# dmlc/difacto

Measured on AMD Instinct MI355X. Metric: examples/sec (FM SGD worker step, Criteo-shape, V_dim=64), higher is better.
Workload: dtype f32

## Files before the change

### difacto_amd/csrc/dfh_localize.hip

```cpp
#ifndef DFH_LOCALIZE_HIP_
#define DFH_LOCALIZE_HIP_
#include "dfh_internal.h"

namespace dfh {

constexpr int LOC_OVERSAMPLE = 8;
constexpr int LOC_MAX_BUCKETS = 1024;
constexpr int LOC_BIG_BUCKETS = 4096;
constexpr int LOC_AVG_BUCKET = 384;
constexpr int LOC_MIN_AVG = 48;
constexpr int LOC_MAX_AVG = 700;
constexpr int LOC_LDS_CAP = 1024;
#ifndef DFH_LOC_TILE
#define DFH_LOC_TILE 2048
#endif
#ifndef DFH_LOC_TILE_THREADS
#define DFH_LOC_TILE_THREADS 1024
#endif
constexpr int LOC_TILE = DFH_LOC_TILE;
constexpr int LOC_TILE_THREADS = DFH_LOC_TILE_THREADS;
constexpr int LOC_PER_THREAD = LOC_TILE / LOC_TILE_THREADS;
constexpr int LOC_SORT_THREADS = 256;
constexpr int LOC_EMIT_THREADS = 256;

struct LocView {
  const uint64_t* raw;
  uint32_t n;
  uint64_t max_index;
  int P;
  int bstride;
  int ntiles;
  int force_global;
  int tb;
  uint32_t nrows;
  const uint32_t* offset;
  const uint32_t* rowid;
  uint64_t* smp_key;
  uint32_t* smp_pos;
  uint32_t* smp_rank;
  uint64_t* spl_key;
  uint32_t* spl_pos;
  uint32_t* packed;
  uint32_t* run_off;
  uint32_t* btotal;
  uint32_t* bstart;
  uint64_t* bkeys;
  uint32_t* bpos;
  uint64_t* skeys;
  uint32_t* spos;
  uint64_t* first_key;
  uint64_t* last_key;
  uint32_t* nheads;
  uint32_t* lh;
  uint32_t* split_n;
};

struct SegListsOut {
  uint2* mid;
  SegEnt* mid_ent;
  uint2* hot;
  SegEnt* hot_ent;
  uint2* few;
  SegEnt* few_ent;
};

__device__ __forceinline__ uint64_t make_key(uint64_t id, uint64_t max_index) {
  const uint64_t m = (max_index == ~0ULL) ? (id == ~0ULL ? 0ULL : id) : id % max_index;
  return reverse_bytes(m);
}

constexpr int LOC_XCDS = 8;

__device__ __forceinline__ bool comp_less(uint64_t ka, uint32_t pa, uint64_t kb, uint32_t pb) {
  return ka < kb || (ka == kb && pa < pb);
}

template <bool MAX>
__device__ __forceinline__ uint32_t wave_inclusive(uint32_t x) {
#define DFH_DPP_STEP(ctrl, row_mask)                                                                      \
  {                                                                                                       \
    const uint32_t y = (uint32_t)__builtin_amdgcn_update_dpp(0, (int)x, ctrl, row_mask, 0xf, false);    \
    x = MAX ? max(x, y) : x + y;                                                                          \
  }
  DFH_DPP_STEP(0x111, 0xf)
  DFH_DPP_STEP(0x112, 0xf)
  DFH_DPP_STEP(0x114, 0xf)
  DFH_DPP_STEP(0x118, 0xf)
  DFH_DPP_STEP(0x142, 0xa)
  DFH_DPP_STEP(0x143, 0xc)
#undef DFH_DPP_STEP
  return x;
}

template <bool MAX, int NWAVES>
__device__ __forceinline__ uint32_t block_exclusive(uint32_t val, uint32_t* wtot , uint32_t* total) {
  static_assert(NWAVES <= 64, "one lane per wave");
  const int lane = (int)(threadIdx.x & 63);
  const int w = __builtin_amdgcn_readfirstlane((int)(threadIdx.x >> 6));
  const uint32_t s = wave_inclusive<MAX>(val);
  __syncthreads();
  if (lane == 63) wtot[w] = s;
  __syncthreads();
  const uint32_t x = wave_inclusive<MAX>(lane < NWAVES ? wtot[lane] : 0u);
  const uint32_t before = w ? (uint32_t)__builtin_amdgcn_readlane((int)x, w - 1) : 0u;
  if (total) *total = (uint32_t)__builtin_amdgcn_readlane((int)x, NWAVES - 1);
  const uint32_t prev = (uint32_t)__builtin_amdgcn_update_dpp(0, (int)s, 0x138, 0xf, 0xf, false);
  return MAX ? max(before, prev) : before + prev;
}
template <int NWAVES>
__device__ __forceinline__ uint32_t block_exclusive_scan(uint32_t val, uint32_t* wsum , uint32_t* total) {
  return block_exclusive<false, NWAVES>(val, wsum, total);
}
template <int NWAVES>
__device__ __forceinline__ uint32_t block_exclusive_max(uint32_t val, uint32_t* wmax , uint32_t* total) {
  return block_exclusive<true, NWAVES>(val, wmax, total);
}

__device__ __forceinline__ uint32_t ss_sample_pos(uint32_t t, uint32_t stride, uint32_t n) {
  const uint32_t j = (uint32_t)(splitmix64(t) >> 33) % stride;
  return min(t * stride + j, n - 1);
}

__global__ void __launch_bounds__(256) k_ss_sample(LocView v) {
  const uint32_t S = (uint32_t)v.P * LOC_OVERSAMPLE;
  const uint32_t stride = max(1u, v.n / S);
  for (uint32_t t = blockIdx.x * blockDim.x + threadIdx.x; t < S; t += gridDim.x * blockDim.x) {
    const uint32_t i = ss_sample_pos(t, stride, v.n);
    v.smp_key[t] = make_key(v.raw[i], v.max_index);
    v.smp_pos[t] = i << v.tb;
    v.smp_rank[t] = 0;
  }
}

__global__ void __launch_bounds__(256) k_ss_rank(LocView v) {
  __shared__ uint64_t ck[256];
  __shared__ uint32_t cp[256];
  const uint32_t S = (uint32_t)v.P * LOC_OVERSAMPLE;
  const uint32_t ntile = (S + 255) / 256;
  const uint32_t ti = blockIdx.x / ntile, tj = blockIdx.x % ntile;
  const uint32_t col = tj * 256 + threadIdx.x;
  ck[threadIdx.x] = col < S ? v.smp_key[col] : ~0ULL;
  cp[threadIdx.x] = col < S ? v.smp_pos[col] : ~0u;
  const uint32_t row = ti * 256 + threadIdx.x;
  const uint64_t mk = row < S ? v.smp_key[row] : 0;
  const uint32_t mp = row < S ? v.smp_pos[row] : 0;
  __syncthreads();
  const uint32_t lim = min(256u, S - tj * 256);
  uint32_t rank = 0;
#pragma unroll 8
  for (uint32_t j = 0; j < lim; ++j) {
    const bool less = comp_less(ck[j], cp[j], mk, mp) || (ck[j] == mk && cp[j] == mp && tj * 256 + j < row);
    rank += less ? 1u : 0u;
  }
  if (row < S && rank) atomicAdd(&v.smp_rank[row], rank);
}

__global__ void __launch_bounds__(256) k_loc_splitters(LocView v) {
  const uint32_t S = (uint32_t)v.P * LOC_OVERSAMPLE;
  for (uint32_t t = blockIdx.x * blockDim.x + threadIdx.x; t < S; t += gridDim.x * blockDim.x) {
    const uint32_t r = v.smp_rank[t];
    if (r > 0 && r % LOC_OVERSAMPLE == 0) {
      v.spl_key[r / LOC_OVERSAMPLE - 1] = v.smp_key[t];
      v.spl_pos[r / LOC_OVERSAMPLE - 1] = v.smp_pos[t];
    }
  }
}

constexpr int LOC_GATHER_ROWS = 1024;
constexpr int LOC_GATHER_SEGS = 4;
struct GatherSrc {
  int nseg;
  uint32_t seg_row0[LOC_GATHER_SEGS + 1];
  const uint32_t* src_off[LOC_GATHER_SEGS];
  const uint64_t* src_idx[LOC_GATHER_SEGS];
  const float* src_val[LOC_GATHER_SEGS];
  const uint32_t* h_rows;
  const uint32_t* h_off;
  const float* h_lab;
  const uint32_t* h_tile_row;
  uint64_t* dst_raw;
  float* dst_val;
  uint32_t* dst_off;
  float* dst_lab;
};
constexpr size_t loc_gather_smem() { return (size_t)(LOC_GATHER_ROWS + 1) * 4 + 4 + (size_t)LOC_GATHER_ROWS * 8; }
template <typename T>
__device__ __forceinline__ T loc_sel(const T (&a)[LOC_GATHER_SEGS], uint32_t sg) {
  T r = a[0];
#pragma unroll
  for (int x = 1; x < LOC_GATHER_SEGS; ++x) r = sg == (uint32_t)x ? a[x] : r;
  return r;
}

template <int MAXB>
constexpr size_t loc_count_smem() { return (size_t)MAXB * 16; }
template <int MAXB, int THREADS>
constexpr size_t loc_scatter_smem() { return (size_t)MAXB * 4 + (THREADS / 64) * 4; }
constexpr size_t loc_sort_smem() { return (size_t)LOC_LDS_CAP * 24 + 2 * (LOC_SORT_THREADS / 64) * 4; }
constexpr size_t loc_emit_smem() { return (2 * (LOC_EMIT_THREADS / 64) + 4) * 4; }

template <int MAXB, int THREADS, bool GATHER = false>
__device__ __forceinline__ void loc_count_block(const LocView& v, const uint32_t bid, const uint32_t nblk, char* smem,
                                                const GatherSrc* gp = nullptr) {
  constexpr int PER = LOC_TILE / THREADS;
  static_assert(PER * THREADS == LOC_TILE, "a tile is a whole number of elements per thread");
  uint64_t* sk = reinterpret_cast<uint64_t*>(smem);
  uint32_t* sp = reinterpret_cast<uint32_t*>(smem + (size_t)MAXB * 8);
  uint32_t* hist = sp + MAXB;
  const int P = v.P;
  for (int b = threadIdx.x; b < P; b += THREADS) {
    hist[b] = 0;
    sk[b] = b < P - 1 ? v.spl_key[b] : ~0ULL;
    sp[b] = b < P - 1 ? v.spl_pos[b] : ~0u;
  }
  const uint32_t base = bid * LOC_TILE;
  if (bid == 0 && threadIdx.x == 0 && v.split_n) *v.split_n = 0u;
  uint64_t key[PER];
  if (GATHER) {
    const GatherSrc& g = *gp;
    uint32_t* roff = reinterpret_cast<uint32_t*>(smem + loc_count_smem<MAXB>());
    uint64_t* rsrc = reinterpret_cast<uint64_t*>(roff + LOC_GATHER_ROWS + 2);
    const uint32_t row0 = g.h_tile_row[bid], row1 = g.h_tile_row[bid + 1];
    const uint32_t nr = min(row1, v.nrows - 1u) - row0 + 1u;
    for (uint32_t q = threadIdx.x; q <= nr; q += THREADS) roff[q] = g.h_off[row0 + q];
    for (uint32_t q = threadIdx.x; q < nr; q += THREADS) {
      const uint32_t r = row0 + q;
      uint32_t sg = 0;
#pragma unroll
      for (int x = 1; x < LOC_GATHER_SEGS; ++x) sg += (x < g.nseg && r >= g.seg_row0[x]) ? 1u : 0u;
      rsrc[q] = ((uint64_t)loc_sel(g.src_off, sg)[g.h_rows[r]] << 2) | sg;
    }
    __syncthreads();
#pragma unroll
    for (int e = 0; e < PER; ++e) {
      const uint32_t i = base + e * THREADS + threadIdx.x;
      key[e] = ~0ULL;
      if (i < v.n) {
        uint32_t lo = 0, hi = nr - 1u;
        while (lo < hi) {
          const uint32_t mid = (lo + hi + 1u) >> 1;
          if (roff[mid] <= i) lo = mid; else hi = mid - 1u;
        }
        const uint64_t sw = rsrc[lo];
        const uint32_t sg = (uint32_t)(sw & 3u);
        const size_t at = (size_t)(sw >> 2) + (i - roff[lo]);
        const uint64_t id = loc_sel(g.src_idx, sg)[at];
        g.dst_raw[i] = id;
        if (g.dst_val) {
          const float* sv = loc_sel(g.src_val, sg);
          g.dst_val[i] = sv ? sv[at] : 1.0f;
        }
        key[e] = make_key(id, v.max_index);
      }
    }
  } else {
#pragma unroll
    for (int e = 0; e < PER; ++e) {
      const uint32_t i = base + e * THREADS + threadIdx.x;
      key[e] = i < v.n ? make_key(v.raw[i], v.max_index) : ~0ULL;
    }
  }
  {
    uint32_t* __restrict__ rowid = const_cast<uint32_t*>(v.rowid);
    const uint32_t* __restrict__ offset = GATHER ? gp->h_off : v.offset;
    const uint32_t rpb = (v.nrows + nblk - 1) / nblk;
    const uint32_t r0 = bid * rpb, r1 = min(v.nrows, r0 + rpb);
    for (uint32_t r = r0 + threadIdx.x; r < r1; r += THREADS) {
      const uint32_t b0 = offset[r], e = offset[r + 1];
      if (GATHER) {
        gp->dst_off[r] = b0;
        gp->dst_lab[r] = gp->h_lab[r];
        if (r + 1 == v.nrows) gp->dst_off[r + 1] = e;
      }
      for (uint32_t j = b0; j < e; ++j) rowid[j] = r;
    }
  }
  __syncthreads();
  int lo[PER], hi[PER];
#pragma unroll
  for (int e = 0; e < PER; ++e) { lo[e] = 0; hi[e] = P - 1; }
  for (int step = P; step > 1; step = (step + 1) >> 1) {
#pragma unroll
    for (int e = 0; e < PER; ++e) {
      if (lo[e] < hi[e]) {
        const uint32_t i = base + e * THREADS + threadIdx.x;
        const int mid = (lo[e] + hi[e]) >> 1;
        if (comp_less(key[e], i << v.tb, sk[mid], sp[mid])) hi[e] = mid; else lo[e] = mid + 1;
      }
    }
  }
#pragma unroll
  for (int e = 0; e < PER; ++e) {
    const uint32_t i = base + e * THREADS + threadIdx.x;
    if (i < v.n) {
      const uint32_t r = atomicAdd(&hist[lo[e]], 1u);
      v.packed[i] = ((uint32_t)lo[e] << 16) | r;
    }
  }
  __syncthreads();
  for (int b = threadIdx.x; b < P; b += THREADS) {
    const uint32_t h = hist[b];
    v.run_off[bid * P + b] = h ? atomicAdd(&v.btotal[(bid & (LOC_XCDS - 1)) * MAXB + b], h) : 0u;
  }
}

template <int MAXB>
__global__ void __launch_bounds__(LOC_TILE_THREADS) k_loc_count(LocView v) {
  __shared__ __attribute__((aligned(16))) char smem[loc_count_smem<MAXB>()];
  loc_count_block<MAXB, LOC_TILE_THREADS>(v, blockIdx.x, gridDim.x, smem);
}
template <int MAXB>
__global__ void __launch_bounds__(LOC_TILE_THREADS) k_loc_count_gather(LocView v, GatherSrc g) {
  __shared__ __attribute__((aligned(16))) char smem[loc_count_smem<MAXB>() + loc_gather_smem()];
  loc_count_block<MAXB, LOC_TILE_THREADS, true>(v, blockIdx.x, gridDim.x, smem, &g);
}

constexpr int LOC_DESC_ROWS = 256;
__global__ void __launch_bounds__(LOC_DESC_ROWS) k_loc_describe(const uint32_t* __restrict__ src_off, const float* __restrict__ src_lab,
                                                                const uint32_t* __restrict__ h_rows, const uint32_t* __restrict__ h_base,
                                                                uint32_t n, uint32_t* __restrict__ dst_off, float* __restrict__ dst_lab,
                                                                int write_end) {
  __shared__ uint32_t wsum[LOC_DESC_ROWS / 64];
  const uint32_t q = blockIdx.x * LOC_DESC_ROWS + threadIdx.x;
  const bool in = q < n;
  const uint32_t r = h_rows[in ? q : n - 1u];
  const uint32_t lo = src_off[r], hi = src_off[r + 1u];
  const float lab = src_lab[r];
  const uint32_t len = in ? hi - lo : 0u;
  const uint32_t at = h_base[blockIdx.x] + block_exclusive_scan<LOC_DESC_ROWS / 64>(len, wsum, nullptr);
  if (in) {
    dst_off[q] = at;
    dst_lab[q] = lab;
    if (write_end && q + 1u == n) dst_off[n] = at + len;
  }
}


template <int MAXB, int THREADS>
__device__ __forceinline__ void loc_scatter_block(const LocView& v, const uint32_t bid, char* smem) {
  constexpr int PER = LOC_TILE / THREADS;
  constexpr int LOC_BPT = MAXB / THREADS;
  static_assert(LOC_BPT * THREADS == MAXB, "the scan of the bucket totals gives every thread the same number of buckets");
  uint32_t* off = reinterpret_cast<uint32_t*>(smem);
  uint32_t* wsum = off + MAXB;
  const int P = v.P;
  const uint32_t xcd = bid & (LOC_XCDS - 1);
  const uint32_t base = bid * LOC_TILE;
  const int b0 = threadIdx.x * LOC_BPT;
  uint32_t tt[LOC_BPT], ro[LOC_BPT];
  uint32_t sum = 0;
#pragma unroll
  for (int q = 0; q < LOC_BPT; ++q) {
    const int bb = min(b0 + q, P - 1);
    const uint32_t in = b0 + q < P ? 1u : 0u;
    tt[q] = 0;
    ro[q] = v.run_off[bid * P + bb];
#pragma unroll
    for (int x = 0; x < LOC_XCDS; ++x) {
      const uint32_t h = v.btotal[x * MAXB + bb];
      tt[q] += h;
      ro[q] += (x < (int)xcd ? 1u : 0u) * h;
    }
    tt[q] *= in;
    ro[q] *= in;
    sum += tt[q];
  }
  uint32_t total;
  uint32_t ex = block_exclusive_scan<THREADS / 64>(sum, wsum, &total);
#pragma unroll
  for (int q = 0; q < LOC_BPT; ++q) {
    if (b0 + q < P) {
      off[b0 + q] = ex + ro[q];
      if (bid == 0) v.bstart[b0 + q] = ex;
    }
    ex += tt[q];
  }
  if (bid == 0 && threadIdx.x == 0) v.bstart[P] = total;
  uint64_t raw[PER];
  uint32_t pk[PER], rw[PER];
#pragma unroll
  for (int e = 0; e < PER; ++e) {
    const uint32_t i = min(base + e * THREADS + threadIdx.x, v.n - 1);
    raw[e] = v.raw[i];
    pk[e] = v.packed[i];
    rw[e] = v.rowid[i];
  }
  __syncthreads();
#pragma unroll
  for (int e = 0; e < PER; ++e) {
    const uint32_t i = base + e * THREADS + threadIdx.x;
    if (i < v.n) {
      const uint32_t dst = off[pk[e] >> 16] + (pk[e] & 0xFFFFu);
      v.bkeys[dst] = make_key(raw[e], v.max_index);
      v.bpos[dst] = (i << v.tb) | (rw[e] & ((1u << v.tb) - 1u));
    }
  }
}

template <int MAXB>
__global__ void __launch_bounds__(LOC_TILE_THREADS) k_loc_scatter(LocView v) {
  __shared__ __attribute__((aligned(16))) char smem[loc_scatter_smem<MAXB, LOC_TILE_THREADS>()];
  loc_scatter_block<MAXB, LOC_TILE_THREADS>(v, blockIdx.x, smem);
}

template <int J>
__device__ __forceinline__ uint32_t loc_net_partner(uint32_t x) {
  static_assert(J == 1 || J == 2 || J == 4 || J == 8, "DPP reaches the partners inside a row of 16 lanes");
  if constexpr (J == 1) return (uint32_t)__builtin_amdgcn_mov_dpp((int)x, 0xB1, 0xf, 0xf, false);
  if constexpr (J == 2) return (uint32_t)__builtin_amdgcn_mov_dpp((int)x, 0x4E, 0xf, 0xf, false);
  if constexpr (J == 4) {
    const int y = __builtin_amdgcn_mov_dpp((int)x, 0x141, 0xf, 0xf, false);
    return (uint32_t)__builtin_amdgcn_mov_dpp(y, 0x1B, 0xf, 0xf, false);
  }
  return (uint32_t)__builtin_amdgcn_mov_dpp((int)x, 0x128, 0xf, 0xf, false);
}
constexpr uint64_t loc_net_keeps_max(int K, int J) {
  uint64_t m = 0;
  for (int i = 0; i < 64; ++i) m |= (uint64_t)(((i & J) != 0) != ((i & K) != 0)) << i;
  return m;
}
template <int K, int J>
__device__ __forceinline__ void loc_net_stage(uint32_t& klo, uint32_t& khi, uint32_t& tag) {
  uint32_t mlo, mhi;
  asm volatile("s_mov_b32 %0, %2\n\ts_mov_b32 %1, %3"
               : "=s"(mlo), "=s"(mhi)
               : "i"((int32_t)(uint32_t)loc_net_keeps_max(K, J)), "i"((int32_t)(uint32_t)(loc_net_keeps_max(K, J) >> 32)));
  const uint64_t mask = ((uint64_t)mhi << 32) | mlo;
  const bool keeps_max = __builtin_amdgcn_inverse_ballot_w64(mask);
  if constexpr (J >= 16) {
    uint32_t alo, ahi, at, blo, bhi, bt;
#define DFH_NET_SWAP(a, b, x)                                                                                       \
    {                                                                                                                 \
      const auto r = J == 16 ? __builtin_amdgcn_permlane16_swap(x, x, false, false) : __builtin_amdgcn_permlane32_swap(x, x, false, false); \
      a = r[0];                                                                                                       \
      b = r[1];                                                                                                       \
    }
    DFH_NET_SWAP(alo, blo, klo)
    DFH_NET_SWAP(ahi, bhi, khi)
    DFH_NET_SWAP(at, bt, tag)
#undef DFH_NET_SWAP
    const bool out_of_order = comp_less(((uint64_t)bhi << 32) | blo, bt, ((uint64_t)ahi << 32) | alo, at);
    const bool take_b = out_of_order != keeps_max;
    klo = take_b ? blo : alo;
    khi = take_b ? bhi : ahi;
    tag = take_b ? bt : at;
  } else {
    const uint32_t olo = loc_net_partner<J>(klo), ohi = loc_net_partner<J>(khi), ot = loc_net_partner<J>(tag);
    const bool partner_less = comp_less(((uint64_t)ohi << 32) | olo, ot, ((uint64_t)khi << 32) | klo, tag);
    const bool take = partner_less != keeps_max;
    klo = take ? olo : klo;
    khi = take ? ohi : khi;
    tag = take ? ot : tag;
  }
}
template <int K, int J>
__device__ __forceinline__ void loc_net_merge(uint32_t& klo, uint32_t& khi, uint32_t& tag) {
  loc_net_stage<K, J>(klo, khi, tag);
  if constexpr (J > 1) loc_net_merge<K, J / 2>(klo, khi, tag);
}
template <int K = 2>
__device__ __forceinline__ void loc_net_sort64(uint32_t& klo, uint32_t& khi, uint32_t& tag) {
  loc_net_merge<K, K / 2>(klo, khi, tag);
  if constexpr (K < 64) loc_net_sort64<K * 2>(klo, khi, tag);
}

__device__ __forceinline__ bool loc_sort_bucket_lds(const LocView& v, uint32_t beg, uint32_t n, uint64_t* ak, uint32_t* ap,
                                                    uint64_t* bk, uint32_t* bp) {
  const uint64_t* gk = v.bkeys + beg;
  const uint32_t* gp = v.bpos + beg;
  uint64_t* sk = bk;
  uint32_t* sp = bp;
  const uint32_t lane = threadIdx.x & 63;
  for (uint32_t c0 = (threadIdx.x >> 6) * 64; c0 < n; c0 += LOC_SORT_THREADS) {
    const uint32_t idx = c0 + lane;
    const bool valid = idx < n;
    const uint64_t mk = valid ? gk[idx] : ~0ULL;
    uint32_t klo = (uint32_t)mk, khi = (uint32_t)(mk >> 32);
    uint32_t mp = valid ? gp[idx] : ~0u;
    loc_net_sort64(klo, khi, mp);
    if (valid) {
      bk[idx] = ((uint64_t)khi << 32) | klo;
      bp[idx] = mp;
    }
  }
  __syncthreads();
  constexpr int E = LOC_LDS_CAP / LOC_SORT_THREADS;
  constexpr int G = 2;
  static_assert(E * LOC_SORT_THREADS == LOC_LDS_CAP && E % G == 0 && LOC_SORT_THREADS % 64 == 0,
                "a thread carries E elements of a full bucket, G at a time");
  uint64_t* dk = ak;
  uint32_t* dp = ap;
  uint32_t sh = 6;
  for (uint32_t L = 64; L < n; L <<= 1, ++sh) {
    for (int g = 0; g < E && g * LOC_SORT_THREADS < (int)n; g += G) {
      uint64_t mk[G];
      uint32_t mp[G], at[G], end[G];
#pragma unroll
      for (int e = 0; e < G; ++e) {
        const uint32_t idx = threadIdx.x + (g + e) * LOC_SORT_THREADS;
        const bool valid = idx < n;
        const uint32_t sib = ((idx >> sh) ^ 1u) << sh;
        mk[e] = valid ? sk[idx] : 0ULL;
        mp[e] = valid ? sp[idx] : 0u;
        at[e] = min(sib, n);
        end[e] = valid ? min(sib + L, n) : at[e];
      }
      for (uint32_t step = L; step; step >>= 1) {
        uint64_t ok[G];
        uint32_t op[G];
#pragma unroll
        for (int e = 0; e < G; ++e) {
          const uint32_t q = at[e] + step <= end[e] ? at[e] + step - 1u : 0u;
          ok[e] = sk[q];
          op[e] = sp[q];
        }
#pragma unroll
        for (int e = 0; e < G; ++e)
          if (at[e] + step <= end[e] && comp_less(ok[e], op[e], mk[e], mp[e])) at[e] += step;
      }
#pragma unroll
      for (int e = 0; e < G; ++e) {
        const uint32_t idx = threadIdx.x + (g + e) * LOC_SORT_THREADS;
        if (idx < n) {
          const uint32_t dst = idx + at[e] - min((idx & ~(L - 1u)) | L, n);
          dk[dst] = mk[e];
          dp[dst] = mp[e];
        }
      }
    }
    __syncthreads();
    uint64_t* tk = sk; sk = dk; dk = tk;
    uint32_t* tp = sp; sp = dp; dp = tp;
  }
  return sk == ak;
}
__device__ __forceinline__ void loc_sort_bucket_global(const LocView& v, uint32_t beg, uint32_t n) {
  uint64_t* xk = v.bkeys + beg;
  uint32_t* xp = v.bpos + beg;
  uint64_t* yk = v.skeys + beg;
  uint32_t* yp = v.spos + beg;
  const uint32_t lane = threadIdx.x & 63;
  for (uint32_t c0 = (threadIdx.x >> 6) * 64; c0 < n; c0 += LOC_SORT_THREADS) {
    const uint32_t idx = c0 + lane;
    const bool valid = idx < n;
    const uint64_t mk = valid ? xk[idx] : ~0ULL;
    const uint32_t mp = valid ? xp[idx] : ~0u;
    const uint32_t lim = min(64u, n - c0);
    uint32_t rank = 0;
    for (uint32_t j = 0; j < lim; ++j) rank += comp_less(xk[c0 + j], xp[c0 + j], mk, mp) ? 1u : 0u;
    if (valid) {
      yk[c0 + rank] = mk;
      yp[c0 + rank] = mp;
    }
  }
  __syncthreads();
  uint64_t* srck = yk; uint32_t* srcp = yp;
  uint64_t* dstk = xk; uint32_t* dstp = xp;
  for (uint32_t L = 64; L < n; L <<= 1) {
    for (uint32_t idx = threadIdx.x; idx < n; idx += blockDim.x) {
      const uint64_t mk = srck[idx];
      const uint32_t mp = srcp[idx];
      const uint32_t r = idx / L;
      const uint32_t pair_base = (r & ~1u) * L;
      const uint32_t sib = (r ^ 1u) * L;
      uint32_t lo = min(sib, n), hi = min(sib + L, n);
      const uint32_t sib_beg = lo;
      while (lo < hi) {
        const uint32_t mid = (lo + hi) >> 1;
        if (comp_less(srck[mid], srcp[mid], mk, mp)) lo = mid + 1; else hi = mid;
      }
      const uint32_t dst = pair_base + (idx - r * L) + (lo - sib_beg);
      dstk[dst] = mk;
      dstp[dst] = mp;
    }
    __syncthreads();
    uint64_t* tk = srck; srck = dstk; dstk = tk;
    uint32_t* tp = srcp; srcp = dstp; dstp = tp;
  }
  if (srck != yk) {
    for (uint32_t t = threadIdx.x; t < n; t += blockDim.x) {
      yk[t] = srck[t];
      yp[t] = srcp[t];
    }
  }
  __syncthreads();
}

struct BucketSummary {
  uint32_t nheads, lh;
  uint64_t first_key, last_key;
};
template <bool WRITE>
__device__ __forceinline__ BucketSummary loc_bucket_summary(const uint64_t* sk, const uint32_t* sp, uint32_t n, uint64_t* ok,
                                                            uint32_t* op, uint32_t (*red)[LOC_SORT_THREADS / 64]) {
  uint32_t cnt = 0, last = 0;
  uint32_t t0 = threadIdx.x;
  asm volatile("" : "+v"(t0));
  for (uint32_t t = t0; t < n; t += LOC_SORT_THREADS) {
    const uint64_t k = sk[t];
    if (WRITE) {
      ok[t] = k;
      op[t] = sp[t];
    }
    if (t + 1 < n && sk[t + 1] != k) {
      ++cnt;
      last = t + 1;
    }
  }
  cnt = (uint32_t)__builtin_amdgcn_readlane((int)wave_inclusive<false>(cnt), 63);
  last = (uint32_t)__builtin_amdgcn_readlane((int)wave_inclusive<true>(last), 63);
  if ((threadIdx.x & 63) == 0) {
    red[0][threadIdx.x >> 6] = cnt;
    red[1][threadIdx.x >> 6] = last;
  }
  __syncthreads();
  BucketSummary r;
  r.nheads = 1;
  r.lh = 0;
  r.first_key = 0;
  r.last_key = 0;
  if (threadIdx.x == 0) {
    for (int w = 0; w < LOC_SORT_THREADS / 64; ++w) {
      r.nheads += red[0][w];
      r.lh = max(r.lh, red[1][w]);
    }
    r.first_key = sk[0];
    r.last_key = sk[n - 1];
  }
  return r;
}

__device__ __forceinline__ void loc_sort_block(const LocView& v, const uint32_t bid, const uint32_t nblk, char* smem) {
  uint64_t* ak = reinterpret_cast<uint64_t*>(smem);
  uint64_t* bk = ak + LOC_LDS_CAP;
  uint32_t* ap = reinterpret_cast<uint32_t*>(bk + LOC_LDS_CAP);
  uint32_t* bp = ap + LOC_LDS_CAP;
  uint32_t (*red)[LOC_SORT_THREADS / 64] = reinterpret_cast<uint32_t (*)[LOC_SORT_THREADS / 64]>(bp + LOC_LDS_CAP);
  for (uint32_t b = bid; b < (uint32_t)v.P; b += nblk) {
    __syncthreads();
    const uint32_t beg = v.bstart[b], end = v.bstart[b + 1];
    const uint32_t n = end - beg;
    if (threadIdx.x < LOC_XCDS) v.btotal[threadIdx.x * v.bstride + b] = 0;
    if (n == 0) {
      if (threadIdx.x == 0) {
        v.nheads[b] = 0;
        v.lh[b] = 0;
        v.first_key[b] = 0;
        v.last_key[b] = 0;
      }
      continue;
    }
    BucketSummary sm;
    if (n <= LOC_LDS_CAP && !v.force_global) {
      const bool in_a = loc_sort_bucket_lds(v, beg, n, ak, ap, bk, bp);
      sm = loc_bucket_summary<true>(in_a ? ak : bk, in_a ? ap : bp, n, v.skeys + beg, v.spos + beg, red);
    } else {
      loc_sort_bucket_global(v, beg, n);
      sm = loc_bucket_summary<false>(v.skeys + beg, v.spos + beg, n, nullptr, nullptr, red);
    }
    if (threadIdx.x == 0) {
      v.nheads[b] = sm.nheads;
      v.lh[b] = sm.lh;
      v.first_key[b] = sm.first_key;
      v.last_key[b] = sm.last_key;
    }
  }
}
__global__ void __launch_bounds__(LOC_SORT_THREADS) k_loc_sort(LocView v) {
  extern __shared__ __attribute__((aligned(16))) char smem[];
  loc_sort_block(v, blockIdx.x, gridDim.x, smem);
}

template <int NW, bool PROBE>
__device__ __forceinline__ void loc_emit_bucket(const LocView& v, uint32_t b, uint32_t beg, uint32_t n, const uint64_t* sk,
                                                const uint32_t* sp, uint32_t cont, uint32_t ubase, uint32_t carry1,
                                                const float* __restrict__ value,
                                                uint64_t* __restrict__ feaids, uint32_t* __restrict__ col_ptr,
                                                uint32_t* __restrict__ index, uint32_t* __restrict__ s_row,
                                                float* __restrict__ s_val, uint32_t* __restrict__ d_U, const SegListsOut& sl,
                                                uint32_t* wsum, uint32_t* wmax, uint32_t* n_mid, uint32_t* n_hot,
                                                uint32_t* n_few, const TableView& tab, uint32_t* __restrict__ urow) {
  const uint32_t P = (uint32_t)v.P;
  const uint32_t moff = beg / (BWD_SMALL + 1) + 2 * b, hoff = beg / (BWD_MID + 1) + 2 * b, foff = beg / 2 + 2 * b;
  uint32_t run_heads = 0, run_max1 = carry1;
  for (uint32_t base = 0; base < n; base += blockDim.x) {
    const uint32_t t = base + threadIdx.x;
    const uint32_t i = beg + t;
    const bool valid = t < n;
    uint64_t key = 0;
    uint32_t tag = 0;
    bool head = false;
    if (valid) {
      key = sk[t];
      tag = sp[t];
      head = t == 0 ? !cont : key != sk[t - 1];
    }
    const uint32_t pos = tag >> v.tb;
    uint32_t nh, mx;
    const uint32_t ex = block_exclusive_scan<NW>(head ? 1u : 0u, wsum, &nh);
    const uint32_t pm = block_exclusive_max<NW>(head ? i + 1 : 0u, wmax, &mx);
    if (valid) {
      const uint32_t incl = run_heads + ex + (head ? 1u : 0u);
      const uint32_t uid = ubase + incl - 1;
      const uint32_t prev1 = max(run_max1, pm);
      if (head) {
        feaids[uid] = key;
        col_ptr[uid] = i;
        if (PROBE) urow[uid] = find_or_insert(tab, key);
        if (prev1) {
          const uint32_t len = i - (prev1 - 1);
          const SegEnt e = make_uint4(uid - 1, prev1 - 1, i, 0u);
          if (len > BWD_MID) sl.hot_ent[hoff + atomicAdd(n_hot, 1u)] = e;
          else if (len > BWD_SMALL) sl.mid_ent[moff + atomicAdd(n_mid, 1u)] = e;
          else if (len > 1) sl.few_ent[foff + atomicAdd(n_few, 1u)] = e;
        }
      }
      index[pos] = uid;
      uint32_t row = tag & ((1u << v.tb) - 1u);
      {
        const uint32_t step = 1u << v.tb;
        uint32_t lo = 0, hi = v.nrows > row ? (v.nrows - 1u - row) >> v.tb : 0u;
        while (lo < hi) {
          const uint32_t mid = (lo + hi + 1u) >> 1;
          if (v.offset[row + mid * step] <= pos) lo = mid; else hi = mid - 1u;
        }
        row += lo * step;
      }
      s_row[i] = row;
      if (value) s_val[i] = value[pos];
      if (i == v.n - 1) {
        *d_U = uid + 1;
        col_ptr[uid + 1] = v.n;
        const uint32_t lbeg = head ? i : prev1 - 1, len = v.n - lbeg;
        const SegEnt e = make_uint4(uid, lbeg, v.n, 0u);
        if (len > BWD_MID) sl.hot_ent[hoff + atomicAdd(n_hot, 1u)] = e;
        else if (len > BWD_SMALL) sl.mid_ent[moff + atomicAdd(n_mid, 1u)] = e;
        else if (len > 1) sl.few_ent[foff + atomicAdd(n_few, 1u)] = e;
      }
    }
    run_heads += nh;
    run_max1 = max(run_max1, mx);
  }
  if (P > 1) {
    const uint64_t N = v.n;
    const uint64_t m0 = max((uint64_t)beg * P / N + ((uint64_t)beg * P % N ? 1u : 0u), (uint64_t)1);
    const uint64_t e1 = (uint64_t)(beg + n) * P;
    const uint64_t m1 = min(e1 / N + (e1 % N ? 1u : 0u), (uint64_t)P);
    for (uint64_t m = m0 + threadIdx.x; m < m1; m += blockDim.x) {
      const uint32_t i = (uint32_t)(m * N / P);
      if ((i * (uint64_t)P + N - 1) / N == m) {
        v.spl_key[m - 1] = sk[i - beg];
        v.spl_pos[m - 1] = sp[i - beg];
      }
    }
  }
  __syncthreads();
  if (threadIdx.x == 0) {
    sl.mid[b] = make_uint2(*n_mid, moff);
    sl.hot[b] = make_uint2(*n_hot, hoff);
    sl.few[b] = make_uint2(*n_few, foff);
  }
}

struct EmitOut {
  const float* value;
  uint64_t* feaids;
  uint32_t* col_ptr;
  uint32_t* index;
  uint32_t* s_row;
  float* s_val;
  uint32_t* d_U;
  SegListsOut sl;
};

template <bool PROBE>
__device__ __forceinline__ void loc_emit_block(const LocView& v, const EmitOut& o, const TableView& tab, uint32_t* __restrict__ urow,
                                               const uint32_t bid, const uint32_t nblk, char* smem) {
  constexpr int NW = LOC_EMIT_THREADS / 64;
  uint32_t* wsum = reinterpret_cast<uint32_t*>(smem);
  uint32_t* wmax = wsum + NW;
  uint32_t& sh_cont = wmax[NW];
  uint32_t& n_mid = wmax[NW + 1];
  uint32_t& n_hot = wmax[NW + 2];
  uint32_t& n_few = wmax[NW + 3];
  const SegListsOut& sl = o.sl;
  const uint32_t P = (uint32_t)v.P;
  for (uint32_t b = bid; b < P; b += nblk) {
    __syncthreads();
    const uint32_t beg = v.bstart[b], end = v.bstart[b + 1];
    const uint32_t n = end - beg;
    if (threadIdx.x == 0) {
      n_mid = 0;
      n_hot = 0;
      n_few = 0;
      if (n == 0) {
        sl.mid[b] = make_uint2(0u, 0u);
        sl.hot[b] = make_uint2(0u, 0u);
        sl.few[b] = make_uint2(0u, 0u);
      }
    }
    if (n == 0) continue;
    uint32_t part = 0, carry1 = 0;
    for (uint32_t q0 = threadIdx.x; q0 <= b; q0 += LOC_EMIT_THREADS) {
      const uint32_t bq = v.bstart[q0], nq = v.bstart[q0 + 1] - bq;
      if (nq == 0) continue;
      int p = (int)q0 - 1;
      while (p >= 0 && v.bstart[p + 1] == v.bstart[p]) --p;
      const uint32_t c = (p >= 0 && v.first_key[q0] == v.last_key[p]) ? 1u : 0u;
      if (q0 == b) {
        sh_cont = c;
      } else {
        part += v.nheads[q0] - c;
        const uint32_t l = v.lh[q0];
        if (l > 0) carry1 = max(carry1, bq + l + 1);
        else if (!c) carry1 = max(carry1, bq + 1);
      }
    }
    uint32_t ubase, carry_all;
    block_exclusive_scan<NW>(part, wsum, &ubase);
    block_exclusive_max<NW>(carry1, wmax, &carry_all);
    __syncthreads();
    loc_emit_bucket<NW, PROBE>(v, b, beg, n, v.skeys + beg, v.spos + beg, sh_cont, ubase, carry_all, o.value, o.feaids, o.col_ptr,
                               o.index, o.s_row, o.s_val, o.d_U, sl, wsum, wmax, &n_mid, &n_hot, &n_few, tab, urow);
  }
}

template <bool PROBE>
__global__ void __launch_bounds__(LOC_EMIT_THREADS) k_loc_emit(LocView v, EmitOut o, TableView tab, uint32_t* __restrict__ urow) {
  __shared__ __attribute__((aligned(16))) char smem[loc_emit_smem()];
  loc_emit_block<PROBE>(v, o, tab, urow, blockIdx.x, gridDim.x, smem);
}

}
#endif
```

Baseline: 87.34 million.

## Sort 128-element runs per wave and merge all runs by rank in one pass

The in-LDS bucket sort now runs a two-register-per-lane bitonic network over 128-element runs instead of 64, with the cross-register stage done in-lane. The log-depth pairwise merge passes, each ending in a block barrier, are replaced by a single pass. In that pass each element finds its final position by binary-searching every other sorted run, then scatters directly to the output buffer. This removes the repeated merge rounds and barriers, but the per-element search cost now grows with the number of runs and padded sentinel entries are written to LDS.

```diff
diff --git a/difacto_amd/csrc/dfh_localize.hip b/difacto_amd/csrc/dfh_localize.hip
--- a/difacto_amd/csrc/dfh_localize.hip
+++ b/difacto_amd/csrc/dfh_localize.hip
@@ -419,14 +419,8 @@
   for (int i = 0; i < 64; ++i) m |= (uint64_t)(((i & J) != 0) != ((i & K) != 0)) << i;
   return m;
 }
-template <int K, int J>
-__device__ __forceinline__ void loc_net_stage(uint32_t& klo, uint32_t& khi, uint32_t& tag) {
-  uint32_t mlo, mhi;
-  asm volatile("s_mov_b32 %0, %2\n\ts_mov_b32 %1, %3"
-               : "=s"(mlo), "=s"(mhi)
-               : "i"((int32_t)(uint32_t)loc_net_keeps_max(K, J)), "i"((int32_t)(uint32_t)(loc_net_keeps_max(K, J) >> 32)));
-  const uint64_t mask = ((uint64_t)mhi << 32) | mlo;
-  const bool keeps_max = __builtin_amdgcn_inverse_ballot_w64(mask);
+template <int J, bool INV>
+__device__ __forceinline__ void loc_net_exchange(const bool keeps_max, uint32_t& klo, uint32_t& khi, uint32_t& tag) {
   if constexpr (J >= 16) {
     uint32_t alo, ahi, at, blo, bhi, bt;
 #define DFH_NET_SWAP(a, b, x)                                                                                       \
@@ -440,99 +434,119 @@
     DFH_NET_SWAP(at, bt, tag)
 #undef DFH_NET_SWAP
     const bool out_of_order = comp_less(((uint64_t)bhi << 32) | blo, bt, ((uint64_t)ahi << 32) | alo, at);
-    const bool take_b = out_of_order != keeps_max;
+    const bool take_b = INV ? out_of_order == keeps_max : out_of_order != keeps_max;
     klo = take_b ? blo : alo;
     khi = take_b ? bhi : ahi;
     tag = take_b ? bt : at;
   } else {
     const uint32_t olo = loc_net_partner<J>(klo), ohi = loc_net_partner<J>(khi), ot = loc_net_partner<J>(tag);
     const bool partner_less = comp_less(((uint64_t)ohi << 32) | olo, ot, ((uint64_t)khi << 32) | klo, tag);
-    const bool take = partner_less != keeps_max;
+    const bool take = INV ? partner_less == keeps_max : partner_less != keeps_max;
     klo = take ? olo : klo;
     khi = take ? ohi : khi;
     tag = take ? ot : tag;
   }
 }
 template <int K, int J>
-__device__ __forceinline__ void loc_net_merge(uint32_t& klo, uint32_t& khi, uint32_t& tag) {
-  loc_net_stage<K, J>(klo, khi, tag);
-  if constexpr (J > 1) loc_net_merge<K, J / 2>(klo, khi, tag);
+__device__ __forceinline__ void loc_net_stage(uint32_t& k0lo, uint32_t& k0hi, uint32_t& t0, uint32_t& k1lo, uint32_t& k1hi,
+                                              uint32_t& t1) {
+  if constexpr (J == 64) {
+    const bool swap = comp_less(((uint64_t)k1hi << 32) | k1lo, t1, ((uint64_t)k0hi << 32) | k0lo, t0);
+    const uint32_t lo = k0lo, hi = k0hi, t = t0;
+    k0lo = swap ? k1lo : lo;
+    k0hi = swap ? k1hi : hi;
+    t0 = swap ? t1 : t;
+    k1lo = swap ? lo : k1lo;
+    k1hi = swap ? hi : k1hi;
+    t1 = swap ? t : t1;
+  } else {
+    uint32_t mlo, mhi;
+    asm volatile("s_mov_b32 %0, %2\n\ts_mov_b32 %1, %3"
+                 : "=s"(mlo), "=s"(mhi)
+                 : "i"((int32_t)(uint32_t)loc_net_keeps_max(K, J)), "i"((int32_t)(uint32_t)(loc_net_keeps_max(K, J) >> 32)));
+    const uint64_t mask = ((uint64_t)mhi << 32) | mlo;
+    const bool keeps_max = __builtin_amdgcn_inverse_ballot_w64(mask);
+    loc_net_exchange<J, false>(keeps_max, k0lo, k0hi, t0);
+    loc_net_exchange<J, K == 64>(keeps_max, k1lo, k1hi, t1);
+  }
+}
+template <int K, int J>
+__device__ __forceinline__ void loc_net_merge(uint32_t& k0lo, uint32_t& k0hi, uint32_t& t0, uint32_t& k1lo, uint32_t& k1hi,
+                                              uint32_t& t1) {
+  loc_net_stage<K, J>(k0lo, k0hi, t0, k1lo, k1hi, t1);
+  if constexpr (J > 1) loc_net_merge<K, J / 2>(k0lo, k0hi, t0, k1lo, k1hi, t1);
 }
 template <int K = 2>
-__device__ __forceinline__ void loc_net_sort64(uint32_t& klo, uint32_t& khi, uint32_t& tag) {
-  loc_net_merge<K, K / 2>(klo, khi, tag);
-  if constexpr (K < 64) loc_net_sort64<K * 2>(klo, khi, tag);
-}
-
-__device__ __forceinline__ bool loc_sort_bucket_lds(const LocView& v, uint32_t beg, uint32_t n, uint64_t* ak, uint32_t* ap,
+__device__ __forceinline__ void loc_net_sort128(uint32_t& k0lo, uint32_t& k0hi, uint32_t& t0, uint32_t& k1lo, uint32_t& k1hi,
+                                                uint32_t& t1) {
+  loc_net_merge<K, K / 2>(k0lo, k0hi, t0, k1lo, k1hi, t1);
+  if constexpr (K < 128) loc_net_sort128<K * 2>(k0lo, k0hi, t0, k1lo, k1hi, t1);
+}
+
+constexpr int LOC_RUN = 128;
+__device__ __forceinline__ void loc_sort_bucket_lds(const LocView& v, uint32_t beg, uint32_t n, uint64_t* ak, uint32_t* ap,
                                                     uint64_t* bk, uint32_t* bp) {
   const uint64_t* gk = v.bkeys + beg;
   const uint32_t* gp = v.bpos + beg;
-  uint64_t* sk = bk;
-  uint32_t* sp = bp;
   const uint32_t lane = threadIdx.x & 63;
-  for (uint32_t c0 = (threadIdx.x >> 6) * 64; c0 < n; c0 += LOC_SORT_THREADS) {
-    const uint32_t idx = c0 + lane;
-    const bool valid = idx < n;
-    const uint64_t mk = valid ? gk[idx] : ~0ULL;
-    uint32_t klo = (uint32_t)mk, khi = (uint32_t)(mk >> 32);
-    uint32_t mp = valid ? gp[idx] : ~0u;
-    loc_net_sort64(klo, khi, mp);
-    if (valid) {
-      bk[idx] = ((uint64_t)khi << 32) | klo;
-      bp[idx] = mp;
-    }
-  }
-  __syncthreads();
-  constexpr int E = LOC_LDS_CAP / LOC_SORT_THREADS;
-  constexpr int G = 2;
-  static_assert(E * LOC_SORT_THREADS == LOC_LDS_CAP && E % G == 0 && LOC_SORT_THREADS % 64 == 0,
-                "a thread carries E elements of a full bucket, G at a time");
-  uint64_t* dk = ak;
-  uint32_t* dp = ap;
-  uint32_t sh = 6;
-  for (uint32_t L = 64; L < n; L <<= 1, ++sh) {
-    for (int g = 0; g < E && g * LOC_SORT_THREADS < (int)n; g += G) {
-      uint64_t mk[G];
-      uint32_t mp[G], at[G], end[G];
-#pragma unroll
-      for (int e = 0; e < G; ++e) {
-        const uint32_t idx = threadIdx.x + (g + e) * LOC_SORT_THREADS;
-        const bool valid = idx < n;
-        const uint32_t sib = ((idx >> sh) ^ 1u) << sh;
-        mk[e] = valid ? sk[idx] : 0ULL;
-        mp[e] = valid ? sp[idx] : 0u;
-        at[e] = min(sib, n);
-        end[e] = valid ? min(sib + L, n) : at[e];
-      }
-      for (uint32_t step = L; step; step >>= 1) {
-        uint64_t ok[G];
-        uint32_t op[G];
-#pragma unroll
-        for (int e = 0; e < G; ++e) {
-          const uint32_t q = at[e] + step <= end[e] ? at[e] + step - 1u : 0u;
-          ok[e] = sk[q];
-          op[e] = sp[q];
+  const uint32_t wave = (uint32_t)__builtin_amdgcn_readfirstlane((int)(threadIdx.x >> 6));
+  constexpr uint32_t PASS = LOC_SORT_THREADS / 64 * LOC_RUN;
+  static_assert(LOC_LDS_CAP % LOC_RUN == 0 && LOC_SORT_THREADS % 64 == 0, "whole runs, whole waves");
+  for (uint32_t c0 = wave * LOC_RUN; c0 < n; c0 += PASS) {
+    const uint32_t i0 = c0 + lane, i1 = c0 + 64 + lane;
+    const bool v0 = i0 < n, v1 = i1 < n;
+    const uint64_t m0 = v0 ? gk[i0] : ~0ULL, m1 = v1 ? gk[i1] : ~0ULL;
+    uint32_t k0lo = (uint32_t)m0, k0hi = (uint32_t)(m0 >> 32), k1lo = (uint32_t)m1, k1hi = (uint32_t)(m1 >> 32);
+    uint32_t t0 = v0 ? gp[i0] : ~0u, t1 = v1 ? gp[i1] : ~0u;
+    loc_net_sort128(k0lo, k0hi, t0, k1lo, k1hi, t1);
+    bk[i0] = ((uint64_t)k0hi << 32) | k0lo;
+    bp[i0] = t0;
+    bk[i1] = ((uint64_t)k1hi << 32) | k1lo;
+    bp[i1] = t1;
+  }
+  __syncthreads();
+  constexpr int GR = 2;
+  const uint32_t nruns = (n + LOC_RUN - 1) / LOC_RUN;
+  for (uint32_t c0 = wave * LOC_RUN; c0 < n; c0 += PASS) {
+    for (uint32_t h = 0; h < LOC_RUN && c0 + h < n; h += 64) {
+      const uint32_t idx = c0 + h + lane;
+      const uint64_t mk = bk[idx];
+      const uint32_t mp = bp[idx];
+      uint32_t dst = h + lane;
+      for (uint32_t j = 0; j + 1 < nruns; j += GR) {
+        uint32_t base[GR], at[GR];
+#pragma unroll
+        for (int r = 0; r < GR; ++r) {
+          uint32_t run = c0 / LOC_RUN + 1 + j + r;
+          if (run >= nruns) run -= nruns;
+          base[r] = j + r + 1 < nruns ? run * LOC_RUN : c0;
+          at[r] = base[r];
         }
 #pragma unroll
-        for (int e = 0; e < G; ++e)
-          if (at[e] + step <= end[e] && comp_less(ok[e], op[e], mk[e], mp[e])) at[e] += step;
-      }
-#pragma unroll
-      for (int e = 0; e < G; ++e) {
-        const uint32_t idx = threadIdx.x + (g + e) * LOC_SORT_THREADS;
-        if (idx < n) {
-          const uint32_t dst = idx + at[e] - min((idx & ~(L - 1u)) | L, n);
-          dk[dst] = mk[e];
-          dp[dst] = mp[e];
+        for (int r = 0; r < GR; ++r)
+          if (j + r + 1 < nruns && comp_less(bk[base[r] + LOC_RUN - 1], bp[base[r] + LOC_RUN - 1], mk, mp)) ++dst;
+#pragma unroll
+        for (uint32_t step = LOC_RUN / 2; step; step >>= 1) {
+          uint64_t ok[GR];
+          uint32_t op[GR];
+#pragma unroll
+          for (int r = 0; r < GR; ++r) {
+            ok[r] = bk[at[r] + step - 1u];
+            op[r] = bp[at[r] + step - 1u];
+          }
+#pragma unroll
+          for (int r = 0; r < GR; ++r) at[r] = comp_less(ok[r], op[r], mk, mp) ? at[r] + step : at[r];
         }
-      }
-    }
-    __syncthreads();
-    uint64_t* tk = sk; sk = dk; dk = tk;
-    uint32_t* tp = sp; sp = dp; dp = tp;
-  }
-  return sk == ak;
+#pragma unroll
+        for (int r = 0; r < GR; ++r) dst += j + r + 1 < nruns ? at[r] - base[r] : 0u;
+      }
+      if (idx < n) {
+        ak[dst] = mk;
+        ap[dst] = mp;
+      }
+    }
+  }
+  __syncthreads();
 }
 __device__ __forceinline__ void loc_sort_bucket_global(const LocView& v, uint32_t beg, uint32_t n) {
   uint64_t* xk = v.bkeys + beg;
@@ -652,8 +666,8 @@
     }
     BucketSummary sm;
     if (n <= LOC_LDS_CAP && !v.force_global) {
-      const bool in_a = loc_sort_bucket_lds(v, beg, n, ak, ap, bk, bp);
-      sm = loc_bucket_summary<true>(in_a ? ak : bk, in_a ? ap : bp, n, v.skeys + beg, v.spos + beg, red);
+      loc_sort_bucket_lds(v, beg, n, ak, ap, bk, bp);
+      sm = loc_bucket_summary<true>(ak, ap, n, v.skeys + beg, v.spos + beg, red);
     } else {
       loc_sort_bucket_global(v, beg, n);
       sm = loc_bucket_summary<false>(v.skeys + beg, v.spos + beg, n, nullptr, nullptr, red);
```

After: 88.08 million, median of 6. Within noise of the previous version (+0.8%).
